# prip-lab/MSU-LatentAFIS

Hardware: AMD Instinct MI355X
Metric: latent queries/sec vs 100k rolled gallery (higher is better)
Workload: dtype f32

## Files before the change

msu-latentafis_amd/csrc/afis_api.cpp:

```cpp
#include "afis_ctx.h"
#include "rank_order.h"
#include <algorithm>
#include <vector>

using namespace afis;

namespace afis {
thread_local std::string g_create_error;
}

extern "C" {

int afis_create(afis_ctx** out, const float* codewords, int M, int K, int dsub, int device_id)
{
    if (!out || !codewords) return fail(nullptr, AFIS_EINVAL, "afis_create: null argument");
    *out = nullptr;
    if (M != kM || K != kK || dsub != kDsub) return fail(nullptr, AFIS_EINVAL, "afis_create: only the M=16, K=256, dsub=6 codebook geometry is supported");
    int n_dev = 0;
    if (hipGetDeviceCount(&n_dev) != hipSuccess || n_dev <= 0) return fail(nullptr, AFIS_EDEVICE, "afis_create: no HIP device (this library has no CPU fallback)");
    if (device_id < 0 || device_id >= n_dev) return fail(nullptr, AFIS_EINVAL, "afis_create: device_id out of range");
    hipDeviceProp_t prop;
    if (hipGetDeviceProperties(&prop, device_id) != hipSuccess) return fail(nullptr, AFIS_EDEVICE, "afis_create: hipGetDeviceProperties failed");
    if (strncmp(prop.gcnArchName, "gfx950", 6) != 0)
        return fail(nullptr, AFIS_EDEVICE, std::string("afis_create: kernels are built for gfx950 only, device is ") + prop.gcnArchName);
// ... 92 lines not shown
    lap("done");
    delete c;
}

const char* afis_last_error(const afis_ctx* ctx) { return ctx ? ctx->err.c_str() : g_create_error.c_str(); }

int afis_get_timing(const afis_ctx* ctx, afis_timing* out)
{
    return afis_get_timing2(ctx, out, offsetof(afis_timing, pairs) + sizeof(int64_t));
}

int afis_get_timing2(const afis_ctx* ctx, afis_timing* out, size_t struct_size)
{
    if (!ctx || !out || struct_size < sizeof(float)) return AFIS_EINVAL;
    memcpy(out, &ctx->timing, std::min(struct_size, sizeof(afis_timing)));
    return AFIS_OK;
}

int afis_rank_list(const float* scores, int64_t n, int ref_order, int k, int64_t* idx, float* sc)
{
    if (n < 0 || k < 0 || (n > 0 && !scores) || (k > 0 && !idx)) return fail(nullptr, AFIS_EINVAL, "afis_rank_list: null argument or negative size");
    if (n > 0x7fffffff) return fail(nullptr, AFIS_EINVAL, "afis_rank_list: more than 2^31 - 1 scores");
    std::vector<int> ind;
    rank_list_order(scores, n, ref_order != 0, ind);
    for (int j = 0; j < k; ++j) {
        const bool in = j < n;
        idx[j] = in ? ind[(size_t)j] : -1;
        if (sc) sc[j] = in ? scores[ind[(size_t)j]] : 0.0f;
    }
    return AFIS_OK;
}


int afis_get_option(const afis_ctx* ctx, const char* name, int64_t* value)
{
    if (!ctx || !name || !value) return AFIS_EINVAL;
    const std::string n(name);
    if (n == "adc_variant") *value = ctx->adc_variant;
    else if (n == "bound_cus") *value = (ctx->stream_lo && !ctx->overlap_failed) ? ctx->bound_cus : 0;
    else if (n == "search_timeout_s") *value = ctx->search_timeout_s <= 0 ? 0 : (int64_t)std::ceil(ctx->search_timeout_s);
    else if (n == "search_timeout_ms") *value = ctx->search_timeout_s <= 0 ? 0 : (int64_t)std::llround(ctx->search_timeout_s * 1e3);
    else if (n == "mf_blocks") *value = 2;
    else if (n == "query_batch") *value = ctx->query_batch;
    else if (n == "chunk") *value = ctx->chunk;
    else if (n == "tile_share") *value = ctx->tile_share;
    else if (n == "minu_generic") *value = ctx->minu_generic;
    else if (n == "s3_tie_order") *value = ctx->s3_tie_order;
    else if (n == "ref_tie_order") *value = ctx->s3_tie_order + ctx->s89_tie_order;
    else if (n == "minu_fast_max_latent") *value = rt_class_max_latent(4);
    else if (n == "minu_fast_max_rolled") *value = rt_class_max_rolled(4);
    else if (n == "minu_fast_max_cells") *value = rt_class_simi_floats(4);
    else if (n == "graph_slab_steps_texture") *value = kTexSlabSteps;
    else if (n == "graph_slab_steps_minutiae") *value = kMinuSlabSteps;
    else if (n == "gallery_resident") *value = (int64_t)ctx->res_empty.size();
    else if (n == "gallery_h2d_bytes") *value = ctx->gallery_h2d_bytes;
    else if (n == "subset_device_bytes") *value = (int64_t)subset_device_bytes(ctx);
    else if (n == "subset_gather_us") *value = ctx->subset_gather_us;
    else if (n == "subject_rank_us") *value = ctx->subject_rank_us;
    else if (n == "rank_hits_us") *value = ctx->rank_hits_us;
    else if (n == "rank_cases_us") *value = ctx->rank_cases_us;
    else if (n == "case_fuse_us") *value = ctx->case_fuse_us;
    else if (n == "case_rank_us") *value = ctx->case_rank_us;
    else if (n == "rank_filtered_us") *value = ctx->rank_filtered_us;
    else if (n == "score_stats_us") *value = ctx->score_stats_us;
    else if (n == "normalize_us") *value = ctx->normalize_us;
    else if (n == "rank_positions_us") *value = ctx->rank_positions_us;
    else if (n == "filter_us") *value = ctx->filter_us;
    else if (n == "eligible_classes") *value = ctx->eligible_classes;
    else if (n == "eligible_expand_us") *value = ctx->eligible_expand_us;
    else if (n == "weighted_batch_pseudo") *value = ctx->weighted_batch_pseudo;
    else if (n == "weighted_pseudo_queries") *value = ctx->weighted_pseudo_queries;
    else if (n == "weighted_fold_us") *value = ctx->weighted_fold_us;
    else if (n == "print_gather_us") *value = ctx->print_gather_us;
    else if (n == "print_h2d_bytes") *value = ctx->print_h2d_bytes;
    else if (n == "rank_latents_us") *value = ctx->rank_latents_us;
    else if (n == "corr_pairs_per_launch") *value = ctx->corr_pairs_per_launch;
    else if (n == "correspondences_us") *value = ctx->correspondences_us;
    else if (n == "score_pairs_per_launch") *value = ctx->score_pairs_per_launch;
    else if (n == "score_pairs_us") *value = ctx->score_pairs_us;
    else if (n == "print_pairs_batch_prints") *value = ctx->print_pairs_batch_prints;
    else if (n == "print_pairs_us") *value = ctx->print_pairs_us;
    else if (n == "print_pairs_query_prints") *value = ctx->print_pairs_query_prints;
    else if (n == "cascade_pairs_per_launch") *value = ctx->cascade_pairs_per_launch;
    else if (n == "cascade_stage1_us") *value = ctx->cascade_stage1_us;
    else if (n == "cascade_select_us") *value = ctx->cascade_select_us;
    else if (n == "cascade_stage2_us") *value = ctx->cascade_stage2_us;
    else if (n == "cascade_kept_pairs") *value = ctx->cascade_kept_pairs;
    else if (n == "print_cascade_stage1_us") *value = ctx->print_cascade_stage1_us;
    else if (n == "print_cascade_select_us") *value = ctx->print_cascade_select_us;
    else if (n == "print_cascade_stage2_us") *value = ctx->print_cascade_stage2_us;
    else if (n == "print_cascade_kept_pairs") *value = ctx->print_cascade_kept_pairs;
    else if (n == "mf_stats") *value = ctx->mf_collect_stats;
    else if (n == "rowmax_budget_mb") *value = ctx->rowmax_budget_bytes >> 20;
    else if (n == "lut_dtype") *value = 32;
    else return AFIS_EINVAL;
    return AFIS_OK;
}

int afis_set_option(afis_ctx* ctx, const char* name, int64_t value)
{
    if (!ctx || !name) return AFIS_EINVAL;
    const std::string n(name);
    if (n == "adc_variant") {
        if (value < 0 || value > 9 || value == 4 || value == 5 || (value < 8 && !g_direct_adc_stage))
            return fail(ctx, AFIS_EINVAL, "adc_variant must be 9 (matrix-core bound pass + exact values) or 8 (16-bit LDS-table bound pass + exact values); the direct kernels 0..3, 6, 7 "
                                          "are reference kernels built into libafis_hip_test.so only");
// ... 45 lines not shown
```

msu-latentafis_amd/csrc/afis_device.h:

```cpp
#pragma once
#include <hip/hip_runtime.h>
#include <stdint.h>

#include "score_order.h"

namespace afis {

typedef unsigned long long u64;
constexpr int kM = 16;
constexpr int kK = 256;
constexpr int kDsub = 6;
constexpr int kDes = 96;
constexpr int kTexMax = 1000;
constexpr int kTopTex = 200;
constexpr int kTopMinu = 120;
constexpr int kDistN = 50;
constexpr int kTileRows = 8;
constexpr int kTileFloats = kTileRows * kM * kK;

struct GalleryDev {
    int32_t G = 0;
    const int32_t* minu_off = nullptr;
    const short2*  minu_xy = nullptr;
    const float*   minu_ori = nullptr;
// ... 111 lines not shown
        }
    }
    int m = 0;
    for (int i = n; i > 0; i = from[i]) cuts[m++] = i;
    for (int a = 0, b = m - 1; a < b; ++a, --b) { const int t = cuts[a]; cuts[a] = cuts[b]; cuts[b] = t; }
    *n_cuts = m;
    delete[] best; delete[] from; delete[] cnt;
}
inline size_t minu_fb_ints(size_t n_tasks, size_t G) { return 1 + n_tasks + 8 + 3 * G; }
inline size_t minu_scratch_floats(int max_nL, int max_nR, int s3_tie_order)
{
    const size_t n = ((size_t)(max_nL > 1 ? max_nL : 1) * (size_t)(max_nR > 1 ? max_nR : 1) + 63) / 64 * 64;
    return (s3_tie_order ? 5 : 2) * n + 4096;
}
struct MinuGrid { size_t wg_floats; int n_wg; size_t bytes() const { return wg_floats * 4 * (size_t)n_wg; } };
inline MinuGrid minu_cands_grid(int max_nL, int max_nR, int s3_tie_order)
{
    MinuGrid g{minu_scratch_floats(max_nL, max_nR, s3_tie_order), 1024};
    while (g.n_wg > 64 && g.bytes() > ((size_t)8 << 30)) g.n_wg /= 2;
    return g;
}
inline MinuGrid minu_cands_pairs_grid(int max_nL, int max_nR, int s3_tie_order, int n_cus, size_t lds_bytes_per_wg, size_t scratch_bytes_held, size_t n_pairs)
{
    MinuGrid g{minu_scratch_floats(max_nL, max_nR, s3_tie_order), 1};
    const size_t afford = scratch_bytes_held > ((size_t)1 << 30) ? scratch_bytes_held : (size_t)1 << 30;
    const size_t per_cu = (size_t)(160 << 10) / lds_bytes_per_wg;
    size_t n = (size_t)(n_cus > 1 ? n_cus : 1) * (per_cu > 1 ? per_cu : 1);
    if (afford / (g.wg_floats * 4) < n) n = afford / (g.wg_floats * 4);
    if (n < 1) n = 1;
    if (3 * n_pairs < n) n = 3 * n_pairs;
    g.n_wg = (int)n;
    return g;
}
inline size_t minu_scratch_bytes(const int* max_nL, size_t n_groups, int max_nR, int s3_tie_order)
{
    size_t bytes = 0;
    for (size_t i = 0; i < n_groups; ++i) { const size_t b = minu_cands_grid(max_nL[i], max_nR, s3_tie_order).bytes(); if (b > bytes) bytes = b; }
    return bytes;
}
enum { kDiagFallback = 0,
       kDiagSmall = 1,
       kDiagCandsClk = 4, kDiagCandsWall = 5,
       kDiagBoundClk = 6, kDiagBoundWall = 7,
       kDiagWords = 16 };
constexpr int kTexSlabSteps = 48, kMinuSlabSteps = 32;
constexpr size_t kTexSlabWgBytes = (size_t)((kTopTex + 63) / 64) * kTexSlabSteps * 64 * 5;
constexpr size_t kMinuSlabWgBytes = (size_t)((kTopMinu + 63) / 64) * kMinuSlabSteps * 64 * 5;
inline int graph_texture_grid(long long n_tasks) { return (int)(n_tasks < 16384 ? n_tasks : 16384); }
inline int graph_minutiae_grid(long long n_tasks) { return (int)(n_tasks < 32768 ? n_tasks : 32768); }
inline size_t graph_texture_slab_bytes(long long n_tasks) { return n_tasks > 0 ? (size_t)graph_texture_grid(n_tasks) * kTexSlabWgBytes : 0; }
inline size_t graph_minutiae_slab_bytes(long long n_tasks) { return n_tasks > 0 ? (size_t)graph_minutiae_grid(n_tasks) * kMinuSlabWgBytes : 0; }
hipError_t launch_graph_texture(const QueryDev& q, const GalleryDev& g, const float* table_dist,
                                const float* rm_val, const int32_t* rm_arg, const float* rm_cv, const int32_t* rm_n, float* parts, void* slab, size_t slab_bytes, MinuCand* tap_out, int32_t* tap_n, int tap_stage, hipStream_t stream);
hipError_t launch_minu_cands(const QueryDev& q, const GalleryDev& g, float* scratch, size_t scratch_floats_per_wg, int n_wg,
                             int force_generic, MinuCand* cands, int32_t* cand_n, int32_t* fallback , int max_nL, int max_nR,
                             unsigned long long* diag , hipStream_t stream);
hipError_t launch_graph_minutiae(const QueryDev& q, const GalleryDev& g, const MinuCand* cands, const int32_t* cand_n,
                                 float* parts, short4* corr_out, int32_t* corr_n, void* slab, size_t slab_bytes, MinuCand* tap_out, int32_t* tap_n, int tap_stage, hipStream_t stream, bool join = false);
constexpr int kCorrPairsPerLaunch = 8192;
constexpr int kCorrPairsMax = 1 << 20;
constexpr size_t kCorrBytesPerPair = 2 * 3 * kTopMinu * 8 + 2 * 3 * 4 + 16 + 8;
size_t minu_cands_lds_bytes(int s3_tie_order);
hipError_t launch_minu_cands_pairs(const QueryDev& q, const GalleryDev& g, float* scratch, size_t scratch_floats_per_wg, int n_wg, int s3_tie_order,
                                   const int32_t* pair_tab, int n_pairs, MinuCand* cands, int32_t* cand_n, hipStream_t stream);
hipError_t launch_graph_minutiae_pairs(const QueryDev& q, const GalleryDev& g, const int32_t* pair_tab, int n_pairs, const MinuCand* cands, const int32_t* cand_n,
                                       float* parts, short4* corr_out, int32_t* corr_n, void* slab, size_t slab_bytes, int s89_tie_order, hipStream_t stream);
hipError_t launch_fuse(const QueryDev& q, const GalleryDev& g, const float* parts, float* scores, hipStream_t stream);
constexpr int kScorePairsPerLaunch = 8192;
constexpr int kScorePairsMax = 1 << 20;
constexpr size_t kScorePairBytes = 2 * 3 * kTopMinu * 8 + 2 * 3 * 4 + 16 + 4 + 16;
hipError_t launch_adc_pairs(const QueryDev& q, const GalleryDev& g, const float* codewords, const int32_t* pair_tab, const int32_t* seg, int n_seg,
                            float* rm_val, int32_t* rm_arg, hipStream_t stream);
hipError_t launch_graph_texture_pairs(const QueryDev& q, const GalleryDev& g, const int32_t* pair_tab, int n_pairs, const float* table_dist, const float* rm_val, const int32_t* rm_arg,
                                      float* parts, void* slab, size_t slab_bytes, int s89_tie_order, hipStream_t stream);
hipError_t launch_fuse_pairs(const QueryDev& q, const GalleryDev& g, const int32_t* pair_tab, int n_pairs, const float* parts, float* scores, hipStream_t stream);
constexpr int kCascadePairsPerLaunch = 16384;
constexpr int kCascadePairsMax = 1 << 20;
hipError_t launch_fuse_stage1(const QueryDev& q, const GalleryDev& g, const float* parts, float* scores, hipStream_t stream);
hipError_t launch_cascade_gather(int n_q, int G, int keep, int n_kept, long long index_base, const long long* kept, const int32_t* q_slot, const int32_t* piece_first,
                                 int n_pieces, const int32_t* piece_q0, const float* parts, int32_t* tab, float* pair_parts, hipStream_t stream);
hipError_t launch_cascade_scatter(int n_q, int G, int keep, int n_kept, long long index_base, const long long* kept, const int32_t* q_slot, const float* pair_score,
                                  float* out, hipStream_t stream);
hipError_t launch_cascade_gather_mapped(int n_q, int G_res, int m, int keep, int n_kept, long long index_base, const long long* kept, const int32_t* q_slot,
                                        const int32_t* piece_first, int n_pieces, const int32_t* piece_q0, const int32_t* inv, const float* parts, int32_t* tab,
                                        float* pair_parts, hipStream_t stream);
hipError_t launch_cascade_scatter_mapped(int n_q, int G_res, int m, int keep, int n_kept, long long index_base, const long long* kept, const int32_t* q_slot,
                                         const float* pair_score, const int32_t* inv, const int32_t* row_of, const int32_t* out_col, long long out_rows, long long out_stride,
                                         float* out, hipStream_t stream);

hipError_t launch_topk(const float* scores, int n_q, int G, int k, long long index_base, long long* out_idx, float* out_score, hipStream_t stream);

hipError_t launch_pq_encode(const float* des, long long n, const float* codewords, uint8_t* codes, hipStream_t stream);
hipError_t launch_fragment_tiles(const float* des, const int32_t* off, const int32_t* tile_off, int n_templates, void* frag, hipStream_t stream);
hipError_t launch_compact_ranges(const void* src, void* dst, int elem_bytes, const int32_t* old_off, const int32_t* new_off, int G, long long n_new, hipStream_t stream);
hipError_t launch_splice_ranges(const void* res, const void* stg, void* dst, int elem_bytes, const int32_t* src_tab, const int32_t* new_off, int G, long long n_new, hipStream_t stream);
hipError_t launch_gather_ranges(const void* src, void* dst, int elem_bytes, const int32_t* src_off, const int32_t* sel, const int32_t* dst_off, int n, long long n_out, hipStream_t stream);
hipError_t launch_subset_topk_map(long long* idx, long long n_idx, const long long* map, int n_map, hipStream_t stream);
hipError_t launch_permute_columns(const void* src, void* dst, int elem_bytes, int n_q, int n, const int32_t* pos, hipStream_t stream);
hipError_t launch_subject_best(const float* scores, int n_q, int G, const int32_t* slot_of, const long long* d_global, long long index_base, int S,
                               unsigned long long* best, hipStream_t stream);
hipError_t launch_topk_subjects(const unsigned long long* best, int n_q, int S, const long long* ids, const float* scores, int G, const long long* d_global, long long index_base,
                                int k, long long* out_id, float* out_score, long long* out_best, hipStream_t stream);
constexpr int kRankHitsMax = 4096;
hipError_t launch_rank_hits(const float* scores, int n_q, int G, const unsigned long long* best, int S, const long long* ids, const long long* d_global, long long index_base,
                            uint32_t thr, int cap, long long* out_n, long long* out_a, float* out_score, long long* out_b, hipStream_t stream);
hipError_t launch_transpose_scores(const float* in, float* out, int n_q, int n, hipStream_t stream);
// ... 44 lines not shown
```

msu-latentafis_amd/csrc/graph.hip:

```cpp
#include "afis_device.h"
#include <type_traits>
#include "atan2f_libm.h"
#include "graph_arith.h"
#include "stdsort_order.h"

namespace afis {

#define AFIS_PI 3.1415926

#if defined(AFIS_PHASE_TIMING) && !defined(AFIS_GRAPH_PAIRS_UNIT)
__device__ u64 g_graph_phase[16];
#define GPH_INIT() u64 gph_t0 = __builtin_readcyclecounter()
#define GPH(i) do { if (threadIdx.x == 0) { const u64 t1_ = __builtin_readcyclecounter(); sm.ph[(i)] += t1_ - gph_t0; gph_t0 = t1_; } } while (0)
#define GPH_T0() const u64 gph_k0 = __builtin_readcyclecounter()
#define GPH_K(i) do { if (threadIdx.x == 0) sm.ph[(i)] += __builtin_readcyclecounter() - gph_k0; } while (0)
#define GPH_ZERO() do { if (threadIdx.x < 16) sm.ph[threadIdx.x] = 0; WSYNC(); } while (0)
#define GPH_FLUSH() do { WSYNC(); if (threadIdx.x < 16 && sm.ph[threadIdx.x]) atomicAdd(&g_graph_phase[threadIdx.x], sm.ph[threadIdx.x]); } while (0)
#else
#define GPH_INIT() do {} while (0)
#define GPH(i) do {} while (0)
#define GPH_T0() do {} while (0)
#define GPH_K(i) do {} while (0)
#define GPH_ZERO() do {} while (0)
#define GPH_FLUSH() do {} while (0)
#endif

__device__ __forceinline__ u64 g_make_key(float v, int idx) { return rank_composite(rank_key(v), (uint32_t)idx); }
__device__ __forceinline__ int g_wave_popc(bool p) { return __popcll(__ballot(p)); }
__device__ __forceinline__ int g_lane_prefix(u64 mask) { return __builtin_amdgcn_mbcnt_hi((uint32_t)(mask >> 32), __builtin_amdgcn_mbcnt_lo((uint32_t)mask, 0)); }
#define WSYNC() __syncthreads()

__device__ __forceinline__ int g_wave_max(int x)
{
    x = max(x, __builtin_amdgcn_update_dpp(0, x, 0xB1, 0xf, 0xf, false));
    x = max(x, __builtin_amdgcn_update_dpp(0, x, 0x4E, 0xf, 0xf, false));
    x = max(x, __builtin_amdgcn_update_dpp(0, x, 0x124, 0xf, 0xf, false));
    x = max(x, __builtin_amdgcn_update_dpp(0, x, 0x128, 0xf, 0xf, false));
    x = max(x, __builtin_amdgcn_update_dpp(x, x, 0x142, 0xa, 0xf, false));
    x = max(x, __builtin_amdgcn_update_dpp(x, x, 0x143, 0xc, 0xf, false));
    return __builtin_amdgcn_readlane(x, 63);
}

__device__ __forceinline__ uint32_t g_wave_max_u32(uint32_t x) { return (uint32_t)g_wave_max((int)(x ^ 0x80000000u)) ^ 0x80000000u; }
__device__ __forceinline__ uint32_t g_wave_min_u32(uint32_t x) { return ~g_wave_max_u32(~x); }

__device__ __forceinline__ int g_wave_sum(int x)
{
    x += __builtin_amdgcn_update_dpp(0, x, 0xB1, 0xf, 0xf, false);
    x += __builtin_amdgcn_update_dpp(0, x, 0x4E, 0xf, 0xf, false);
    x += __builtin_amdgcn_update_dpp(0, x, 0x124, 0xf, 0xf, false);
    x += __builtin_amdgcn_update_dpp(0, x, 0x128, 0xf, 0xf, false);
    x += __builtin_amdgcn_update_dpp(0, x, 0x142, 0xa, 0xf, false);
    x += __builtin_amdgcn_update_dpp(0, x, 0x143, 0xc, 0xf, false);
    return __builtin_amdgcn_readlane(x, 63);
}

typedef __amdgpu_buffer_rsrc_t SlabBuf;
typedef uint32_t v4u __attribute__((ext_vector_type(4)));
__device__ __forceinline__ SlabBuf g_slab_buf(unsigned char* base, uint32_t bytes) { return __builtin_amdgcn_make_buffer_rsrc(base, 0, (int)bytes, 0x00020000); }

struct Pt { int lx, ly, rx, ry; };
__device__ __forceinline__ int2 pack_xy(int lx, int ly, int rx, int ry) { return make_int2((lx & 0xffff) | (ly << 16), (rx & 0xffff) | (ry << 16)); }
__device__ __forceinline__ Pt unpack_xy(int2 v) { Pt p; p.lx = (int)(short)v.x; p.ly = v.x >> 16; p.rx = (int)(short)v.y; p.ry = v.y >> 16; return p; }

template <int N, bool OWN> struct SimStore { float simv[N]; };
template <int N> struct SimStore<N, false> {};

#ifndef AFIS_MINU_ALIAS
#define AFIS_MINU_ALIAS 1
#endif
template <int NMAX_, bool OWN_SIM_>
struct __attribute__((aligned(16))) WaveSmem : SimStore<NMAX_, OWN_SIM_> {
    static constexpr int NMAX = NMAX_;
    static constexpr bool OWN_SIM = OWN_SIM_;
    static constexpr bool ALIAS_ORI = NMAX_ > 128 || AFIS_MINU_ALIAS;
    static constexpr int W = (NMAX + 31) / 32;
    static constexpr int N4 = (NMAX + 3) / 4 * 4;
    static constexpr int U = (NMAX + 63) / 64;
    float b[N4];
    union {
        float cc[N4];
        struct { short order[NMAX]; short sel[NMAX]; } os;
    } y;
    short li[NMAX], ri[NMAX];
    int2 xy[NMAX];
    uint32_t hb[NMAX][W];
    union {
        uint32_t sortbuf[N4 + 128];
        struct { u64 keys[N4]; float lo[ALIAS_ORI ? 1 : NMAX], ro[ALIAS_ORI ? 1 : NMAX]; } s;
        struct { uint32_t keys[N4]; short te[NMAX], targ[NMAX]; } pick;
    } x;
#ifdef AFIS_PHASE_TIMING
    u64 ph[16];
#endif
};
template <class SM> __device__ __forceinline__ int l_row(int v) { if constexpr (SM::OWN_SIM) return v; else return v & 1023; }
template <class SM> __device__ __forceinline__ int r_pt(int v) { if constexpr (SM::OWN_SIM) return v; else return v & 1023; }
__device__ __forceinline__ int tex_slot_of(int li, int ri) { return ((li >> 10) & 31) | (((ri >> 10) & 31) << 5); }
__device__ __forceinline__ short tex_pack_l(int row, int slot) { return (short)(row | ((slot & 31) << 10)); }
__device__ __forceinline__ short tex_pack_r(int pt, int slot) { return (short)(pt | ((slot >> 5) << 10)); }
template <class SM>
__device__ __forceinline__ float list_sim(const SM& sm, const float* __restrict__ ext, int t)
{
    if constexpr (SM::OWN_SIM) return sm.simv[t];
    else return ext[tex_slot_of(sm.li[t], sm.ri[t])];
}

__device__ __forceinline__ int next_task(int32_t* ctr)
{
    int t;
    unsigned long long saved;
    asm volatile("s_mov_b64 %1, exec\n\t"
                 "s_mov_b64 exec, 1\n\t"
                 "global_atomic_add %0, %2, %3, %4 sc0\n\t"
                 "s_waitcnt vmcnt(0)\n\t"
                 "s_mov_b64 exec, %1"
                 : "=&v"(t), "=&s"(saved) : "v"(0), "v"(1), "s"(ctr) : "memory");
    return __builtin_amdgcn_readfirstlane(t);
}

template <class SM, int ref_tie>
__device__ __forceinline__ void sort_scores(SM& sm, int num, double thr)
{
    const int lane = threadIdx.x;
    constexpr int U = SM::U;
    uint32_t* const s_key = reinterpret_cast<uint32_t*>(sm.x.s.keys);
    uint32_t* const s_cnt = s_key + SM::N4;
    uint32_t* const s_gkey = reinterpret_cast<uint32_t*>(sm.y.cc);
    static_assert(sizeof(sm.x) >= (size_t)(SM::N4 + 128) * 4, "sort scratch exceeds the union");
    uint32_t m32[U]; int r[U];
    if (num <= 48) {
        const u64 mine = lane < num ? g_make_key(sm.b[lane], lane) : 0ull;
        if (lane < num) sm.x.s.keys[lane] = mine;
        WSYNC();
        int rr = 0;
        for (int k = 0; k < num; ++k) rr += sm.x.s.keys[k] > mine;
        if (ref_tie && num > 16) {
            int gg = 0;
            for (int k = 0; k < num; ++k) gg += (uint32_t)(sm.x.s.keys[k] >> 32) > (uint32_t)(mine >> 32);
            const bool tied = lane < num && gg != rr && !((double)sm.b[lane] < thr);
            if (__ballot(tied) != 0ull) {
                uint32_t* const k32 = reinterpret_cast<uint32_t*>(sm.x.s.keys) + 96;
                static_assert(sizeof(sm.x.s.keys) >= (96 + 48 + 48) * 4, "no room for the keys and the stack of the std::sort restatement");
                WSYNC();
                if (lane < num) { k32[lane] = (uint32_t)(mine >> 32); sm.y.os.order[lane] = (short)lane; }
                WSYNC();
                if (lane == 0) stdsort_prefix<uint16_t>(reinterpret_cast<uint16_t*>(sm.y.os.order), num, num, k32, reinterpret_cast<int*>(k32 + 48));
                WSYNC();
                return;
            }
        }
        WSYNC();
        if (lane < num) sm.y.os.order[rr] = (short)lane;
        WSYNC();
        return;
    }
    uint32_t kmin = 0xffffffffu, kmax = 0u;
#pragma unroll
    for (int u = 0; u < U; ++u) {
        const int t = lane + 64 * u;
        m32[u] = t < num ? rank_key(sm.b[t]) : 0u;
        if (t < num) { s_key[t] = m32[u]; kmin = min(kmin, m32[u]); kmax = max(kmax, m32[u]); }
    }
#pragma unroll
    for (int off = 32; off >= 1; off >>= 1) { kmin = min(kmin, (uint32_t)__shfl_xor((int)kmin, off)); kmax = max(kmax, (uint32_t)__shfl_xor((int)kmax, off)); }
    const uint32_t span = kmax - kmin;
    const int sh = max(0, 26 - __clz((int)(span | 1u)));
    int bin[U];
#pragma unroll
    for (int u = 0; u < U; ++u) bin[u] = (int)((m32[u] - kmin) >> sh) & 63;
    s_cnt[lane] = 0u;
    WSYNC();
#pragma unroll
    for (int u = 0; u < U; ++u) if (lane + 64 * u < num) atomicAdd(&s_cnt[bin[u]], 1u);
    WSYNC();
    {
        const int own = (int)s_cnt[lane];
        int suf = own;
#pragma unroll
        for (int off = 1; off < 64; off <<= 1) { const int v = __shfl_down(suf, off); if (lane + off < 64) suf += v; }
        WSYNC();
        s_cnt[lane] = (uint32_t)(suf - own); s_cnt[64 + lane] = (uint32_t)(suf - own);
    }
    WSYNC();
#pragma unroll
    for (int u = 0; u < U; ++u) if (lane + 64 * u < num) s_gkey[atomicAdd(&s_cnt[bin[u]], 1u)] = m32[u];
    WSYNC();
    int rsum = 0;
#pragma unroll
    for (int u = 0; u < U; ++u) {
        r[u] = 0;
        if (lane + 64 * u < num) {
            const int lo = (int)s_cnt[64 + bin[u]], hi = (int)s_cnt[bin[u]];
            int c = lo;
            for (int k = lo; k < hi; ++k) c += s_gkey[k] > m32[u];
            r[u] = c; rsum += c;
        }
    }
    if (g_wave_sum(rsum) != num * (num - 1) / 2) {
        u64 mine[U];
        int gg[U];
#pragma unroll
        for (int u = 0; u < U; ++u) { const int t = lane + 64 * u; mine[u] = t < num ? ((u64)m32[u] << 32) | (uint32_t)(~(uint32_t)t) : 0ull; r[u] = 0; gg[u] = 0; }
        for (int k = 0; k < num; ++k) {
            const u64 kk = ((u64)s_key[k] << 32) | (uint32_t)(~(uint32_t)k);
#pragma unroll
            for (int u = 0; u < U; ++u) { r[u] += kk > mine[u]; gg[u] += s_key[k] > m32[u]; }
        }
        if (ref_tie) {
            bool tied = false;
#pragma unroll
            for (int u = 0; u < U; ++u) { const int t = lane + 64 * u; tied |= t < num && gg[u] != r[u] && !((double)sm.b[t] < thr); }
            if (__ballot(tied) != 0ull) {
                WSYNC();
#pragma unroll
                for (int u = 0; u < U; ++u) { const int t = lane + 64 * u; if (t < num) sm.y.os.order[t] = (short)t; }
                WSYNC();
                if (lane == 0) stdsort_prefix<uint16_t>(reinterpret_cast<uint16_t*>(sm.y.os.order), num, num, s_key, reinterpret_cast<int*>(s_cnt));
                WSYNC();
                return;
            }
        }
    }
    WSYNC();
#pragma unroll
    for (int u = 0; u < U; ++u) { const int t = lane + 64 * u; if (t < num) sm.y.os.order[r[u]] = (short)t; }
    WSYNC();
}

template <class SM, class Compat>
__device__ int greedy(SM& sm, int num, double thr, Compat compatible)
{
    const int lane = threadIdx.x;
    constexpr int U = SM::U;
    int idx[U], li[U], ri[U];
    bool alive[U];
#pragma unroll
    for (int u = 0; u < U; ++u) {
        const int p = lane + 64 * u;
        idx[u] = 0; li[u] = -1; ri[u] = -1; alive[u] = false;
        if (p < num) {
            idx[u] = sm.y.os.order[p];
            li[u] = l_row<SM>(sm.li[idx[u]]); ri[u] = r_pt<SM>(sm.ri[idx[u]]);
            alive[u] = !((double)sm.b[idx[u]] < thr);
        }
    }
    int nsel = 0;
    for (;;) {
        int first = -1, cidx = 0, cli = 0, cri = 0;
#pragma unroll
        for (int u = 0; u < U; ++u) {
            const u64 m = __ballot(alive[u]);
            if (first < 0 && m) {
                const int fl = __ffsll((long long)m) - 1;
                first = 64 * u + fl;
                cidx = __shfl(idx[u], fl); cli = __shfl(li[u], fl); cri = __shfl(ri[u], fl);
            }
        }
        if (first < 0) break;
        if (lane == 0) sm.y.os.sel[nsel] = (short)cidx;
        ++nsel;
#pragma unroll
        for (int u = 0; u < U; ++u) {
            if (alive[u]) {
                const int p = lane + 64 * u;
                if (p == first || li[u] == cli || ri[u] == cri || !compatible(cidx, idx[u])) alive[u] = false;
            }
        }
    }
    WSYNC();
    return nsel;
// ... 484 lines not shown
        WSYNC();
    }
    GPH(PH + 5);
    sort_scores<SM, REF_TIE>(sm, num, 0.001);
    const int nsel = greedy(sm, num, 0.001, [&sm](int a, int o) { return (sm.hb[a][o >> 5] >> (o & 31)) & 1u; });
    compact(sm, nsel);
    GPH(PH + 6);
    return nsel;
}

template <class SM, bool LOOKUP, int ITERS, int REF_TIE>
__device__ __forceinline__ float graph_score(SM& sm, int num, const float* __restrict__ table, const float* __restrict__ lori,
                                             const float* __restrict__ rori, const float* __restrict__ ext, SlabBuf slab, int& n_survivors, int stop_after = 2, int mode = 0)
{
    n_survivors = num;
    if (stop_after == 0) return 0.0f;
    if (mode == 2 && LOOKUP) num = dist_filter<SM, LOOKUP, ITERS, 2, REF_TIE>(sm, num, table, ext, slab);
    else if (mode >= 1) num = dist_filter<SM, LOOKUP, ITERS, 1, REF_TIE>(sm, num, table, ext, slab);
    else num = dist_filter<SM, LOOKUP, ITERS, 0, REF_TIE>(sm, num, table, ext, slab);
    n_survivors = num;
    if (mode >= 1) {
        for (int t = threadIdx.x; t < num; t += 64) {
            const int2 v = sm.xy[t];
            int lx, ly, rx, ry;
            unpack_h2(v.x, lx, ly); unpack_h2(v.y, rx, ry);
            sm.xy[t] = pack_xy(lx, ly, rx, ry);
        }
        WSYNC();
    }
    if (stop_after == 1) return 0.0f;
    n_survivors = 0;
    if (num < 2) return 0.0f;
    num = angle_filter<SM, REF_TIE>(sm, num, lori, rori);
    n_survivors = num;
    for (int t = threadIdx.x; t < num; t += 64) sm.b[t] = list_sim(sm, ext, t);
    WSYNC();
    float score = 0.0f;
    for (int i = 0; i < num; ++i) score += sm.b[i];
    return score;
}

struct GraphTap { MinuCand* out; int32_t* n; int stage; };
template <class SM>
__device__ __forceinline__ void tap_write(const GraphTap& tap, const SM& sm, const float* __restrict__ ext, long long task, int n, int cap)
{
    for (int t = threadIdx.x; t < n; t += 64) { MinuCand c; c.sim = list_sim(sm, ext, t); c.li = l_row<SM>(sm.li[t]); c.ri = r_pt<SM>(sm.ri[t]); tap.out[(size_t)task * cap + t] = c; }
    if (threadIdx.x == 0) tap.n[task] = n;
}

#ifndef AFIS_TEX_WAVES
#define AFIS_TEX_WAVES 4
#endif
typedef WaveSmem<kTopTex, false> TexSmem;
constexpr int kTexRegs = (kTexMax + 63) / 64;
constexpr int kTexFast = 256;
constexpr int kTexFastRegs = kTexFast / 64;

__device__ __forceinline__ const int32_t* pair_tab_of() { return nullptr; }
__device__ __forceinline__ const int32_t* pair_tab_of(const int32_t* tab) { return tab; }
template <int REF_TIE, class... TAB>
__global__ __launch_bounds__(64) __attribute__((amdgpu_waves_per_eu(AFIS_TEX_WAVES, AFIS_TEX_WAVES))) void k_graph_texture(QueryDev q, GalleryDev g, const float* __restrict__ table_dist,
                                                      const float* __restrict__ rm_val, const int32_t* __restrict__ rm_arg,
                                                      const float* __restrict__ rm_cv, const int32_t* __restrict__ rm_n,
                                                      float* __restrict__ parts, unsigned char* slab_all, GraphTap tap, TAB... tab)
{
    constexpr bool PAIRS = sizeof...(TAB) != 0;
    const int32_t* const ptab = pair_tab_of(tab...);
    __shared__ TexSmem sm;
    const SlabBuf slab = g_slab_buf(slab_all + (size_t)blockIdx.x * kTexSlabWgBytes, (uint32_t)kTexSlabWgBytes);
    const int lane = threadIdx.x;
    GPH_ZERO();
    int n_tasks;
    if constexpr (PAIRS) n_tasks = ptab[0]; else n_tasks = q.nq * g.G;
    for (;;) {
        const int task = next_task(g.task_ctr + 0);
        if (task >= n_tasks) break;
        GPH_T0();
        int qi, gi;
        if constexpr (PAIRS) { qi = ptab[1 + 2 * task]; gi = ptab[2 + 2 * task]; }
        else { qi = task / g.G; gi = task - qi * g.G; }
        const int l0 = q.lt_off[qi], n_lt = q.lt_off[qi + 1] - l0;
        const int r0 = g.tex_off[gi], n_rt = g.tex_off[gi + 1] - r0;
        float* out = parts + (size_t)task * 4 + 3;
        if (n_lt <= 0 || n_rt <= 0) { if (lane == 0) { *out = 0.0f; if (tap.out) tap.n[task] = -1; } continue; }
        const size_t o = (size_t)task * q.lt_pad;
        int num;
        if (n_lt > kTopTex) {
            const bool compact = rm_n != nullptr;
            const int n_in = compact ? rm_n[task] : n_lt;
            if (compact && n_in >= kTopTex && n_in <= kTexFast) {
                uint32_t key[kTexFastRegs]; int arg[kTexFastRegs];
                uint32_t kmin = 0xffffffffu, kmax = 0u;
#pragma unroll
                for (int u = 0; u < kTexFastRegs; ++u) {
                    const int e = u * 64 + lane;
                    const bool in = e < n_in;
                    key[u] = in ? rank_key(rm_cv[o + e]) : 0u;
                    arg[u] = in ? rm_arg[o + e] : 0;
                    kmax = max(kmax, key[u]);
                    if (in) kmin = min(kmin, key[u]);
                }
                kmin = g_wave_min_u32(kmin); kmax = g_wave_max_u32(kmax);
                const int shift = max(0, 27 - __clz((int)((kmax - kmin) >> 1) | 1));
                uint32_t* const s_cnt = reinterpret_cast<uint32_t*>(sm.b);
                uint32_t* const s_gkey = sm.x.sortbuf;
                static_assert(TexSmem::N4 >= 128 && sizeof(sm.x.sortbuf) >= (size_t)kTexFast * 4, "the counting arrays of the compact S7 exceed their buffers");
                int bin[kTexFastRegs], r[kTexFastRegs];
#pragma unroll
                for (int u = 0; u < kTexFastRegs; ++u) bin[u] = min((int)((key[u] - kmin) >> shift), 63);
                s_cnt[lane] = 0u;
                WSYNC();
#pragma unroll
                for (int u = 0; u < kTexFastRegs; ++u) if (u * 64 + lane < n_in) atomicAdd(&s_cnt[bin[u]], 1u);
                WSYNC();
                {
                    const int own = (int)s_cnt[lane];
                    int suf = own;
#pragma unroll
                    for (int off = 1; off < 64; off <<= 1) { const int v = __shfl_down(suf, off); if (lane + off < 64) suf += v; }
                    WSYNC();
                    s_cnt[lane] = (uint32_t)(suf - own); s_cnt[64 + lane] = (uint32_t)(suf - own);
                }
                WSYNC();
#pragma unroll
                for (int u = 0; u < kTexFastRegs; ++u) if (u * 64 + lane < n_in) s_gkey[atomicAdd(&s_cnt[bin[u]], 1u)] = key[u];
                WSYNC();
                int rsum = 0;
#pragma unroll
                for (int u = 0; u < kTexFastRegs; ++u) {
                    r[u] = 0;
                    if (u * 64 + lane < n_in) {
                        const int lo = (int)s_cnt[64 + bin[u]], hi = (int)s_cnt[bin[u]];
                        int c = lo;
                        for (int k = lo; k < hi; ++k) c += s_gkey[k] > key[u];
                        r[u] = c; rsum += c;
                    }
                }
                if (g_wave_sum(rsum) != n_in * (n_in - 1) / 2) {
                    WSYNC();
#pragma unroll
                    for (int u = 0; u < kTexFastRegs; ++u) if (u * 64 + lane < n_in) s_gkey[u * 64 + lane] = key[u];
                    WSYNC();
                    u64 mine[kTexFastRegs];
#pragma unroll
                    for (int u = 0; u < kTexFastRegs; ++u) { mine[u] = ((u64)key[u] << 32) | (uint32_t)(~(uint32_t)(u * 64 + lane)); r[u] = 0; }
                    for (int k = 0; k < n_in; ++k) {
                        const u64 kk = ((u64)s_gkey[k] << 32) | (uint32_t)(~(uint32_t)k);
#pragma unroll
                        for (int u = 0; u < kTexFastRegs; ++u) r[u] += kk > mine[u];
                    }
                }
#pragma unroll
                for (int u = 0; u < kTexFastRegs; ++u) {
                    const int e = u * 64 + lane;
                    if (e < n_in && r[u] < kTopTex) { sm.li[r[u]] = tex_pack_l(arg[u] & 0xffff, e); sm.ri[r[u]] = tex_pack_r(arg[u] >> 16, e); }
                }
                num = kTopTex;
            } else {
                const int n_regs = (n_in + 63) >> 6;
                uint32_t key[kTexRegs]; int arg[kTexRegs];
#pragma unroll
                for (int u = 0; u < kTexRegs; ++u) {
                    const int e = u * 64 + lane;
                    const bool in = e < n_in;
                    key[u] = 0u; arg[u] = 0;
                    if (u < n_regs) {
                        key[u] = in ? rank_key(compact ? rm_cv[o + e] : rm_val[o + e]) : 0u;
                        arg[u] = in ? rm_arg[o + e] : 0;
                    }
                }
                uint32_t T = 0;
                for (int bit = 31; bit >= 0; --bit) {
                    const uint32_t cand = T | (1u << bit);
                    int c = 0;
#pragma unroll
                    for (int u = 0; u < kTexRegs; ++u) if (u < n_regs) c += g_wave_popc(key[u] >= cand);
                    if (c >= kTopTex) { T = cand; if (c == kTopTex) break; }
                }
                int n_gt = 0;
#pragma unroll
                for (int u = 0; u < kTexRegs; ++u) if (u < n_regs) n_gt += g_wave_popc(key[u] > T);
                const int need = kTopTex - n_gt;
                int base_gt = 0, base_eq = 0;
                uint32_t* const key32 = sm.x.pick.keys;
#pragma unroll
                for (int u = 0; u < kTexRegs; ++u) {
                    if (u < n_regs) {
                        const int e = u * 64 + lane;
                        const bool gt = key[u] > T, eq = key[u] == T;
                        const u64 mg = __ballot(gt), me = __ballot(eq);
                        int pos = -1;
                        if (gt) pos = base_gt + g_lane_prefix(mg);
                        else if (eq) { const int r = base_eq + g_lane_prefix(me); if (r < need) pos = n_gt + r; }
                        if (pos >= 0) { key32[pos] = key[u]; sm.x.pick.te[pos] = tex_pack_l(compact ? arg[u] & 0xffff : e, e); sm.x.pick.targ[pos] = tex_pack_r(compact ? arg[u] >> 16 : arg[u], e); }
                        base_gt += __popcll(mg); base_eq += __popcll(me);
                    }
                }
                WSYNC();
                num = kTopTex;
                uint32_t m32[TexSmem::U]; int r[TexSmem::U];
                uint32_t* const s_cnt = reinterpret_cast<uint32_t*>(sm.b);
                uint32_t* const s_gkey = reinterpret_cast<uint32_t*>(sm.y.cc);
                int dmax = 0;
#pragma unroll
                for (int u = 0; u < TexSmem::U; ++u) {
                    const int t = lane + 64 * u;
                    m32[u] = t < num ? key32[t] : T;
                    dmax = max(dmax, (int)((m32[u] - T) >> 1));
                }
                dmax = g_wave_max(dmax);
                const int shift = max(0, 27 - __clz(dmax | 1));
                int bin[TexSmem::U];
#pragma unroll
                for (int u = 0; u < TexSmem::U; ++u) bin[u] = min((int)((m32[u] - T) >> shift), 63);
                s_cnt[lane] = 0u;
                WSYNC();
#pragma unroll
                for (int u = 0; u < TexSmem::U; ++u) if (lane + 64 * u < num) atomicAdd(&s_cnt[bin[u]], 1u);
                WSYNC();
                {
                    const int own = (int)s_cnt[lane];
                    int suf = own;
#pragma unroll
                    for (int off = 1; off < 64; off <<= 1) { const int v = __shfl_down(suf, off); if (lane + off < 64) suf += v; }
                    WSYNC();
                    s_cnt[lane] = (uint32_t)(suf - own); s_cnt[64 + lane] = (uint32_t)(suf - own);
                }
                WSYNC();
#pragma unroll
                for (int u = 0; u < TexSmem::U; ++u) if (lane + 64 * u < num) s_gkey[atomicAdd(&s_cnt[bin[u]], 1u)] = m32[u];
                WSYNC();
#pragma unroll
                for (int u = 0; u < TexSmem::U; ++u) {
                    r[u] = 0;
                    if (lane + 64 * u < num) {
                        const int lo = (int)s_cnt[64 + bin[u]], hi = (int)s_cnt[bin[u]];
                        int c = lo;
                        for (int k = lo; k < hi; ++k) c += s_gkey[k] > m32[u];
                        r[u] = c;
                    }
                }
                int rsum = 0;
#pragma unroll
                for (int u = 0; u < TexSmem::U; ++u) rsum += r[u];
                if (g_wave_sum(rsum) != kTopTex * (kTopTex - 1) / 2) {
                    u64 mine[TexSmem::U];
#pragma unroll
                    for (int u = 0; u < TexSmem::U; ++u) { const int t = lane + 64 * u; mine[u] = t < num ? ((u64)key32[t] << 32) | (uint32_t)(~(uint32_t)(sm.x.pick.te[t] & 1023)) : 0ull; r[u] = 0; }
                    for (int k = 0; k < num; ++k) {
                        const u64 kk = ((u64)key32[k] << 32) | (uint32_t)(~(uint32_t)(sm.x.pick.te[k] & 1023));
#pragma unroll
                        for (int u = 0; u < TexSmem::U; ++u) r[u] += kk > mine[u];
                    }
                }
#pragma unroll
                for (int u = 0; u < TexSmem::U; ++u) {
                    const int t = lane + 64 * u;
                    if (t < num) { sm.li[r[u]] = sm.x.pick.te[t]; sm.ri[r[u]] = sm.x.pick.targ[t]; }
                }
            }
        } else {
            num = n_lt;
            for (int t = lane; t < num; t += 64) { sm.li[t] = tex_pack_l(t, t); sm.ri[t] = tex_pack_r(rm_n ? rm_arg[o + t] >> 16 : rm_arg[o + t], t); }
        }
        WSYNC();
        int out_of_range = 0, not_small = 0;
        short2 lp4[TexSmem::U], rp4[TexSmem::U];
#pragma unroll
        for (int u = 0; u < TexSmem::U; ++u) {
            const int t = lane + 64 * u;
            lp4[u] = make_short2(0, 0); rp4[u] = make_short2(0, 0);
            if (t < num) {
                lp4[u] = q.lt_xy[l0 + (sm.li[t] & 1023)]; rp4[u] = g.tex_xy[r0 + (sm.ri[t] & 1023)];
                out_of_range |= (lp4[u].x | lp4[u].y | rp4[u].x | rp4[u].y) & ~2047;
                not_small |= ((unsigned)lp4[u].x > 49u) | ((unsigned)lp4[u].y > 49u) | ((unsigned)rp4[u].x > 49u) | ((unsigned)rp4[u].y > 49u);
            }
        }
        const int mode = __ballot(out_of_range != 0) != 0ull ? 0 : (__ballot(not_small != 0) == 0ull ? 2 : 1);
#pragma unroll
        for (int u = 0; u < TexSmem::U; ++u) {
            const int t = lane + 64 * u;
            if (t < num) sm.xy[t] = mode ? make_int2(pack_h2(lp4[u].x, lp4[u].y), pack_h2(rp4[u].x, rp4[u].y)) : pack_xy(lp4[u].x, lp4[u].y, rp4[u].x, rp4[u].y);
        }
        WSYNC();
        GPH_K(15);
        int n_surv;
        const float* const row_max = (rm_n ? rm_cv : rm_val) + o;
        const float score = graph_score<TexSmem, true, 3, REF_TIE>(sm, num, table_dist, q.lt_ori + l0, g.tex_ori + r0, row_max, slab, n_surv, tap.out ? tap.stage : 2, mode);
        if (lane == 0) *out = score;
        if (tap.out) tap_write(tap, sm, row_max, task, n_surv, kTopTex);
        WSYNC();
    }
    GPH_FLUSH();
}

#ifndef AFIS_GRAPH_PAIRS_UNIT
hipError_t launch_graph_texture(const QueryDev& q, const GalleryDev& g, const float* table_dist,
                                const float* rm_val, const int32_t* rm_arg, const float* rm_cv, const int32_t* rm_n, float* parts, void* slab, size_t slab_bytes, MinuCand* tap_out, int32_t* tap_n, int tap_stage, hipStream_t stream)
{
    const long long n_tasks = (long long)q.nq * g.G;
    if (n_tasks <= 0) return hipSuccess;
    if (n_tasks > 0x7ffffff0LL || !g.task_ctr) return hipErrorInvalidValue;
    const int grid = graph_texture_grid(n_tasks);
    if (!slab || slab_bytes < (size_t)grid * kTexSlabWgBytes) return hipErrorInvalidValue;
    hipError_t e0 = hipMemsetAsync(g.task_ctr + 0, 0, 4, stream);
    if (e0 != hipSuccess) return e0;
    const GraphTap tap{tap_out, tap_n, tap_stage & 255};
    if ((tap_stage >> 8) & 1) hipLaunchKernelGGL(k_graph_texture<1>, dim3(grid), dim3(64), 0, stream, q, g, table_dist, rm_val, rm_arg, rm_cv, rm_n, parts, (unsigned char*)slab, tap);
    else hipLaunchKernelGGL(k_graph_texture<0>, dim3(grid), dim3(64), 0, stream, q, g, table_dist, rm_val, rm_arg, rm_cv, rm_n, parts, (unsigned char*)slab, tap);
    return hipGetLastError();
}
// ... 140 lines not shown
    return hipGetLastError();
}

__device__ __forceinline__ void arith_check(bool tex, float f1, float f2, unsigned long long* cnt)
{
    const float d = fabsf(sqrt_rn_pos(f1) - sqrt_rn_pos(f2));
    const bool ref = tex ? 16.0f * d < 30.0f : d < 30.0f;
    const int a = tex ? pair_compatible_alg<true>(f1, f2) : pair_compatible_alg<false>(f1, f2);
    const bool full = tex ? pair_compatible_n<true>(f1, f2) : pair_compatible_n<false>(f1, f2);
    atomicAdd(cnt + 0, 1ull);
    if (a == 2) atomicAdd(cnt + 1, 1ull);
    if ((a != 2 && (a == 1) != ref) || full != ref) atomicAdd(cnt + 2, 1ull);
}
__global__ __launch_bounds__(256) void k_debug_graph_arith(int part, unsigned long long* __restrict__ cnt)
{
    constexpr unsigned kMaxN = 2u * 2047u * 2047u;
    if (part == 0) {
        const unsigned n = blockIdx.x * 256u + threadIdx.x;
        if (n <= kMaxN && __float_as_uint(sqrt_rn_int((float)n)) != __float_as_uint(sqrt_rn_pos((float)n))) atomicAdd(cnt, 1ull);
    } else if (part == 3) {
        const int dx = (int)blockIdx.x - 2047, dy = (int)(blockIdx.y * 256u + threadIdx.x) - 2047;
        if (dy > 2047) return;
        const int ax = dx > 0 ? dx : 0, ox = dx > 0 ? 0 : -dx, ay = dy > 0 ? dy : 0, oy = dy > 0 ? 0 : -dy;
        const float n = diff_n(pack_h2(ax, ay), pack_h2(ox, oy));
        int bx, by; unpack_h2(pack_h2(ax, ay), bx, by);
        if (__float_as_uint(n) != __float_as_uint((float)(dx * dx + dy * dy)) || bx != ax || by != ay) atomicAdd(cnt, 1ull);
    } else if (part == 1) {
        const unsigned n1 = blockIdx.x, n2 = blockIdx.y * 256u + threadIdx.x;
        if (n1 <= 4802u && n2 <= 4802u) arith_check(true, (float)n1, (float)n2, cnt + 1);
    } else {
        const unsigned n1 = blockIdx.x * 256u + threadIdx.x;
        if (n1 > kMaxN) return;
        const double a = sqrt((double)n1);
        for (int sg = -1; sg <= 1; sg += 2) {
            const double b = a + 30.0 * sg;
            if (b < 0) continue;
            const long long c = (long long)(b * b + 0.5);
            for (int j = -12; j <= 12; ++j) { const long long n2 = c + j; if (n2 >= 0 && n2 <= (long long)kMaxN) arith_check(false, (float)n1, (float)n2, cnt + 4); }
        }
    }
}
hipError_t launch_debug_graph_arith(unsigned long long* cnt8, hipStream_t stream)
{
    constexpr unsigned kMaxN = 2u * 2047u * 2047u;
    hipError_t e = hipMemsetAsync(cnt8, 0, 64, stream);
    if (e != hipSuccess) return e;
    hipLaunchKernelGGL(k_debug_graph_arith, dim3((kMaxN + 256) / 256), dim3(256), 0, stream, 0, cnt8);
    hipLaunchKernelGGL(k_debug_graph_arith, dim3(4803, 19), dim3(256), 0, stream, 1, cnt8);
    hipLaunchKernelGGL(k_debug_graph_arith, dim3((kMaxN + 256) / 256), dim3(256), 0, stream, 2, cnt8);
    hipLaunchKernelGGL(k_debug_graph_arith, dim3(4095, 16), dim3(256), 0, stream, 3, cnt8 + 7);
    return hipGetLastError();
}

hipError_t read_graph_phase_cycles(unsigned long long* out16, bool reset)
{
#ifdef AFIS_PHASE_TIMING
    hipError_t e = hipMemcpyFromSymbol(out16, HIP_SYMBOL(g_graph_phase), 16 * sizeof(u64));
    if (e != hipSuccess) return e;
    if (reset) { u64 z[16] = {}; e = hipMemcpyToSymbol(HIP_SYMBOL(g_graph_phase), z, sizeof(z)); }
    return e;
#else
    for (int i = 0; i < 16; ++i) out16[i] = 0;
    return hipSuccess;
#endif
}

#endif

}
```

Before: 51.05.

## Shrink texture-graph wave LDS by overlaying sort scratch onto bit rows and cc

Reorganizes the per-wave shared-memory struct so the S7 pick scratch and a new s7key buffer share a union with the hb bit rows. The sort key and count buffers shrink to a small union, and scratch for the rare tie-break paths moves into the cc area or into sm.b, with sm.b saved and restored around the sort. The aim is to fit a texture list's LDS within 10 KB so more waves are resident per CU, and a static_assert enforces that limit. It also adds an occupancy query to the API. The risk is aliasing bugs where buffers that share storage are still live at the same time.

```diff
diff --git a/msu-latentafis_amd/csrc/afis_api.cpp b/msu-latentafis_amd/csrc/afis_api.cpp
--- a/msu-latentafis_amd/csrc/afis_api.cpp
+++ b/msu-latentafis_amd/csrc/afis_api.cpp
@@ -168,6 +168,11 @@
     else if (n == "minu_fast_max_cells") *value = rt_class_simi_floats(4);
     else if (n == "graph_slab_steps_texture") *value = kTexSlabSteps;
     else if (n == "graph_slab_steps_minutiae") *value = kMinuSlabSteps;
+    else if (n == "graph_texture_lists_per_cu") {
+        int lists = 0;
+        if (hipSetDevice(ctx->device) != hipSuccess || graph_texture_lists_per_cu(&lists) != hipSuccess) return AFIS_EDEVICE;
+        *value = lists;
+    }
     else if (n == "gallery_resident") *value = (int64_t)ctx->res_empty.size();
     else if (n == "gallery_h2d_bytes") *value = ctx->gallery_h2d_bytes;
     else if (n == "subset_device_bytes") *value = (int64_t)subset_device_bytes(ctx);
diff --git a/msu-latentafis_amd/csrc/afis_device.h b/msu-latentafis_amd/csrc/afis_device.h
--- a/msu-latentafis_amd/csrc/afis_device.h
+++ b/msu-latentafis_amd/csrc/afis_device.h
@@ -187,6 +187,7 @@
 inline size_t graph_minutiae_slab_bytes(long long n_tasks) { return n_tasks > 0 ? (size_t)graph_minutiae_grid(n_tasks) * kMinuSlabWgBytes : 0; }
 hipError_t launch_graph_texture(const QueryDev& q, const GalleryDev& g, const float* table_dist,
                                 const float* rm_val, const int32_t* rm_arg, const float* rm_cv, const int32_t* rm_n, float* parts, void* slab, size_t slab_bytes, MinuCand* tap_out, int32_t* tap_n, int tap_stage, hipStream_t stream);
+hipError_t graph_texture_lists_per_cu(int* lists);
 hipError_t launch_minu_cands(const QueryDev& q, const GalleryDev& g, float* scratch, size_t scratch_floats_per_wg, int n_wg,
                              int force_generic, MinuCand* cands, int32_t* cand_n, int32_t* fallback , int max_nL, int max_nR,
                              unsigned long long* diag , hipStream_t stream);
diff --git a/msu-latentafis_amd/csrc/graph.hip b/msu-latentafis_amd/csrc/graph.hip
--- a/msu-latentafis_amd/csrc/graph.hip
+++ b/msu-latentafis_amd/csrc/graph.hip
@@ -69,6 +69,7 @@
 #ifndef AFIS_MINU_ALIAS
 #define AFIS_MINU_ALIAS 1
 #endif
+constexpr int kSortShort = 48;
 template <int NMAX_, bool OWN_SIM_>
 struct __attribute__((aligned(16))) WaveSmem : SimStore<NMAX_, OWN_SIM_> {
     static constexpr int NMAX = NMAX_;
@@ -84,11 +85,15 @@
     } y;
     short li[NMAX], ri[NMAX];
     int2 xy[NMAX];
-    uint32_t hb[NMAX][W];
     union {
-        uint32_t sortbuf[N4 + 128];
-        struct { u64 keys[N4]; float lo[ALIAS_ORI ? 1 : NMAX], ro[ALIAS_ORI ? 1 : NMAX]; } s;
+        uint32_t hb[NMAX][W];
         struct { uint32_t keys[N4]; short te[NMAX], targ[NMAX]; } pick;
+        uint32_t s7key[NMAX > 128 ? 256 : 1];
+    };
+    union {
+        uint32_t cnt[128];
+        u64 keys[kSortShort];
+        struct { float lo[ALIAS_ORI ? 1 : NMAX], ro[ALIAS_ORI ? 1 : NMAX]; } s;
     } x;
 #ifdef AFIS_PHASE_TIMING
     u64 ph[16];
@@ -124,28 +129,28 @@
 {
     const int lane = threadIdx.x;
     constexpr int U = SM::U;
-    uint32_t* const s_key = reinterpret_cast<uint32_t*>(sm.x.s.keys);
-    uint32_t* const s_cnt = s_key + SM::N4;
+    uint32_t* const s_cnt = sm.x.cnt;
     uint32_t* const s_gkey = reinterpret_cast<uint32_t*>(sm.y.cc);
-    static_assert(sizeof(sm.x) >= (size_t)(SM::N4 + 128) * 4, "sort scratch exceeds the union");
+    uint32_t* const s_key = s_gkey;
     uint32_t m32[U]; int r[U];
-    if (num <= 48) {
+    if (num <= kSortShort) {
         const u64 mine = lane < num ? g_make_key(sm.b[lane], lane) : 0ull;
-        if (lane < num) sm.x.s.keys[lane] = mine;
+        if (lane < num) sm.x.keys[lane] = mine;
         WSYNC();
         int rr = 0;
-        for (int k = 0; k < num; ++k) rr += sm.x.s.keys[k] > mine;
+        for (int k = 0; k < num; ++k) rr += sm.x.keys[k] > mine;
         if (ref_tie && num > 16) {
             int gg = 0;
-            for (int k = 0; k < num; ++k) gg += (uint32_t)(sm.x.s.keys[k] >> 32) > (uint32_t)(mine >> 32);
+            for (int k = 0; k < num; ++k) gg += (uint32_t)(sm.x.keys[k] >> 32) > (uint32_t)(mine >> 32);
             const bool tied = lane < num && gg != rr && !((double)sm.b[lane] < thr);
             if (__ballot(tied) != 0ull) {
-                uint32_t* const k32 = reinterpret_cast<uint32_t*>(sm.x.s.keys) + 96;
-                static_assert(sizeof(sm.x.s.keys) >= (96 + 48 + 48) * 4, "no room for the keys and the stack of the std::sort restatement");
+                constexpr int kOrd = kSortShort / 2;
+                uint32_t* const k32 = s_gkey + kOrd;
+                static_assert(SM::N4 >= kOrd + 2 * kSortShort, "no room in cc for the keys and the stack of the std::sort restatement");
                 WSYNC();
                 if (lane < num) { k32[lane] = (uint32_t)(mine >> 32); sm.y.os.order[lane] = (short)lane; }
                 WSYNC();
-                if (lane == 0) stdsort_prefix<uint16_t>(reinterpret_cast<uint16_t*>(sm.y.os.order), num, num, k32, reinterpret_cast<int*>(k32 + 48));
+                if (lane == 0) stdsort_prefix<uint16_t>(reinterpret_cast<uint16_t*>(sm.y.os.order), num, num, k32, reinterpret_cast<int*>(k32 + kSortShort));
                 WSYNC();
                 return;
             }
@@ -160,7 +165,7 @@
     for (int u = 0; u < U; ++u) {
         const int t = lane + 64 * u;
         m32[u] = t < num ? rank_key(sm.b[t]) : 0u;
-        if (t < num) { s_key[t] = m32[u]; kmin = min(kmin, m32[u]); kmax = max(kmax, m32[u]); }
+        if (t < num) { kmin = min(kmin, m32[u]); kmax = max(kmax, m32[u]); }
     }
 #pragma unroll
     for (int off = 32; off >= 1; off >>= 1) { kmin = min(kmin, (uint32_t)__shfl_xor((int)kmin, off)); kmax = max(kmax, (uint32_t)__shfl_xor((int)kmax, off)); }
@@ -200,6 +205,10 @@
     if (g_wave_sum(rsum) != num * (num - 1) / 2) {
         u64 mine[U];
         int gg[U];
+        WSYNC();
+#pragma unroll
+        for (int u = 0; u < U; ++u) { const int t = lane + 64 * u; if (t < num) s_key[t] = m32[u]; }
+        WSYNC();
 #pragma unroll
         for (int u = 0; u < U; ++u) { const int t = lane + 64 * u; mine[u] = t < num ? ((u64)m32[u] << 32) | (uint32_t)(~(uint32_t)t) : 0ull; r[u] = 0; gg[u] = 0; }
         for (int k = 0; k < num; ++k) {
@@ -212,11 +221,18 @@
 #pragma unroll
             for (int u = 0; u < U; ++u) { const int t = lane + 64 * u; tied |= t < num && gg[u] != r[u] && !((double)sm.b[t] < thr); }
             if (__ballot(tied) != 0ull) {
-                WSYNC();
-#pragma unroll
-                for (int u = 0; u < U; ++u) { const int t = lane + 64 * u; if (t < num) sm.y.os.order[t] = (short)t; }
-                WSYNC();
-                if (lane == 0) stdsort_prefix<uint16_t>(reinterpret_cast<uint16_t*>(sm.y.os.order), num, num, s_key, reinterpret_cast<int*>(s_cnt));
+                uint32_t* const bkey = reinterpret_cast<uint32_t*>(sm.b);
+                float keep[U];
+#pragma unroll
+                for (int u = 0; u < U; ++u) { const int t = lane + 64 * u; keep[u] = t < num ? sm.b[t] : 0.0f; }
+                WSYNC();
+#pragma unroll
+                for (int u = 0; u < U; ++u) { const int t = lane + 64 * u; if (t < num) { sm.y.os.order[t] = (short)t; bkey[t] = m32[u]; } }
+                WSYNC();
+                if (lane == 0) stdsort_prefix<uint16_t>(reinterpret_cast<uint16_t*>(sm.y.os.order), num, num, bkey, reinterpret_cast<int*>(s_cnt));
+                WSYNC();
+#pragma unroll
+                for (int u = 0; u < U; ++u) { const int t = lane + 64 * u; if (t < num) sm.b[t] = keep[u]; }
                 WSYNC();
                 return;
             }
@@ -807,6 +823,8 @@
 #define AFIS_TEX_WAVES 4
 #endif
 typedef WaveSmem<kTopTex, false> TexSmem;
+static_assert(sizeof(TexSmem) <= 10240, "a texture list's LDS exceeds a sixteenth of a CU's: two of the CU's 16 wave slots would stay empty");
+static_assert(sizeof(TexSmem::pick) <= sizeof(TexSmem::hb), "S7's scratch exceeds the bit rows it borrows");
 constexpr int kTexRegs = (kTexMax + 63) / 64;
 constexpr int kTexFast = 256;
 constexpr int kTexFastRegs = kTexFast / 64;
@@ -858,8 +876,8 @@
                 kmin = g_wave_min_u32(kmin); kmax = g_wave_max_u32(kmax);
                 const int shift = max(0, 27 - __clz((int)((kmax - kmin) >> 1) | 1));
                 uint32_t* const s_cnt = reinterpret_cast<uint32_t*>(sm.b);
-                uint32_t* const s_gkey = sm.x.sortbuf;
-                static_assert(TexSmem::N4 >= 128 && sizeof(sm.x.sortbuf) >= (size_t)kTexFast * 4, "the counting arrays of the compact S7 exceed their buffers");
+                uint32_t* const s_gkey = sm.s7key;
+                static_assert(TexSmem::N4 >= 128 && sizeof(sm.s7key) >= (size_t)kTexFast * 4 && sizeof(sm.s7key) <= sizeof(sm.hb), "the counting arrays of the compact S7 exceed their buffers");
                 int bin[kTexFastRegs], r[kTexFastRegs];
 #pragma unroll
                 for (int u = 0; u < kTexFastRegs; ++u) bin[u] = min((int)((key[u] - kmin) >> shift), 63);
@@ -937,7 +955,7 @@
                 for (int u = 0; u < kTexRegs; ++u) if (u < n_regs) n_gt += g_wave_popc(key[u] > T);
                 const int need = kTopTex - n_gt;
                 int base_gt = 0, base_eq = 0;
-                uint32_t* const key32 = sm.x.pick.keys;
+                uint32_t* const key32 = sm.pick.keys;
 #pragma unroll
                 for (int u = 0; u < kTexRegs; ++u) {
                     if (u < n_regs) {
@@ -947,7 +965,7 @@
                         int pos = -1;
                         if (gt) pos = base_gt + g_lane_prefix(mg);
                         else if (eq) { const int r = base_eq + g_lane_prefix(me); if (r < need) pos = n_gt + r; }
-                        if (pos >= 0) { key32[pos] = key[u]; sm.x.pick.te[pos] = tex_pack_l(compact ? arg[u] & 0xffff : e, e); sm.x.pick.targ[pos] = tex_pack_r(compact ? arg[u] >> 16 : arg[u], e); }
+                        if (pos >= 0) { key32[pos] = key[u]; sm.pick.te[pos] = tex_pack_l(compact ? arg[u] & 0xffff : e, e); sm.pick.targ[pos] = tex_pack_r(compact ? arg[u] >> 16 : arg[u], e); }
                         base_gt += __popcll(mg); base_eq += __popcll(me);
                     }
                 }
@@ -1001,9 +1019,9 @@
                 if (g_wave_sum(rsum) != kTopTex * (kTopTex - 1) / 2) {
                     u64 mine[TexSmem::U];
 #pragma unroll
-                    for (int u = 0; u < TexSmem::U; ++u) { const int t = lane + 64 * u; mine[u] = t < num ? ((u64)key32[t] << 32) | (uint32_t)(~(uint32_t)(sm.x.pick.te[t] & 1023)) : 0ull; r[u] = 0; }
+                    for (int u = 0; u < TexSmem::U; ++u) { const int t = lane + 64 * u; mine[u] = t < num ? ((u64)key32[t] << 32) | (uint32_t)(~(uint32_t)(sm.pick.te[t] & 1023)) : 0ull; r[u] = 0; }
                     for (int k = 0; k < num; ++k) {
-                        const u64 kk = ((u64)key32[k] << 32) | (uint32_t)(~(uint32_t)(sm.x.pick.te[k] & 1023));
+                        const u64 kk = ((u64)key32[k] << 32) | (uint32_t)(~(uint32_t)(sm.pick.te[k] & 1023));
 #pragma unroll
                         for (int u = 0; u < TexSmem::U; ++u) r[u] += kk > mine[u];
                     }
@@ -1011,7 +1029,7 @@
 #pragma unroll
                 for (int u = 0; u < TexSmem::U; ++u) {
                     const int t = lane + 64 * u;
-                    if (t < num) { sm.li[r[u]] = sm.x.pick.te[t]; sm.ri[r[u]] = sm.x.pick.targ[t]; }
+                    if (t < num) { sm.li[r[u]] = sm.pick.te[t]; sm.ri[r[u]] = sm.pick.targ[t]; }
                 }
             }
         } else {
@@ -1258,6 +1276,11 @@
     return hipGetLastError();
 }
 
+hipError_t graph_texture_lists_per_cu(int* lists)
+{
+    return hipOccupancyMaxActiveBlocksPerMultiprocessor(lists, k_graph_texture<0>, 64, 0);
+}
+
 hipError_t read_graph_phase_cycles(unsigned long long* out16, bool reset)
 {
 #ifdef AFIS_PHASE_TIMING
```

After: 51.85, median of 6. 1.02x the previous value.
